# Desilo/liberate-fhe

Measured on AMD Instinct MI355X. Metric: NTTs/sec (forward negacyclic poly-NTT, logN=16, L=30 limbs, bit-exact vs reference semantics), higher is better.
Workload: dtype int64; 1 GPU; gold preset (logN=16), rows 9..38 of the prime chain (25 scale + base + 4 special primes = 30 limbs), 128 polynomials per GPU per step, forward NTT via lf_ntt_ws (C ABI: lf_ntt through a resident workspace of the operands' size); workspace_bytes=2013511680, batch_per_gpu=128, limbs=30, logN=16, parallelism=replicas x1 (independent polynomials)

## Files before the change

liberate_fhe_amd/csrc/ckks_ntt_core.h:

```cpp
#pragma once
#include "ckks_common.h"
#include <stdlib.h>

#define NTT_THREADS 512
#define NTT_PASS_WAVES 6
#define NTT_LDS_WORDS ((1 << NTT_TILE_LOG_MAX) + (1 << (NTT_TILE_LOG_MAX - 3)))
#define TAIL_NONE (-1)
#define SMALL_PRIME_LIMIT (1ull << SMALL_PRIME_BITS)

#define PAD(L) ((L) + ((L) >> 3))
#define PAD_STRIDE(LOGDL) ((1 << (LOGDL)) + ((1 << (LOGDL)) >> 3))
#define NTT_FLAG_WORD NTT_LDS_WORDS

namespace {

__device__ __forceinline__ int lf_tid() {
    const int wave = __builtin_amdgcn_readfirstlane((int)threadIdx.x >> 6);
    int lane;
    asm volatile("v_mbcnt_lo_u32_b32 %0, -1, 0\n\tv_mbcnt_hi_u32_b32 %0, -1, %0" : "=v"(lane));
    return (wave << 6) | lane;
}

__device__ __forceinline__ void lds_barrier() {
    asm volatile("s_waitcnt lgkmcnt(0)" ::: "memory");
// ... 512 lines not shown
    int s = g.s0, left = g.S, log_d = g.strided ? g.logC : 0;
    Ctx cc = c;
    int nstep = 0;
    auto arm = [&](int K) {
        ++nstep;
        cc.inv_reduce = ((nstep & 1) == 0) || (left - K <= 0);
    };
    if (FAST && g.tl == 12 && g.S == 12) {
        StepTwInv<A, 0> t0;
        StepTwInv<A, 3> t3;
        StepTwInv<A, 6> t6;
        StepTwInv<A, 9> t9;
        t0.load(c, s, adj, g.logN, base, lf_tid());
        arm(3); inv_step8<A, 0>(sm, t0, cc, lf_tid()); left -= 3;
        t3.load(c, s + 3, adj, g.logN, base, lf_tid());
        lds_barrier();
        arm(3); inv_step8<A, 3>(sm, t3, cc, lf_tid()); left -= 3;
        t6.load(c, s + 6, adj, g.logN, base, lf_tid());
        lds_barrier();
        arm(3); inv_step8<A, 6>(sm, t6, cc, lf_tid()); left -= 3;
        t9.load(c, s + 9, adj, g.logN, base, lf_tid());
        lds_barrier();
        arm(3); inv_step8<A, 9>(sm, t9, cc, lf_tid());
        lds_barrier();
        return;
    }
    while (left > 0) {
        if (FAST && left >= 3) {
            arm(3);
            inv_step<3, A>(sm, T, log_d, s, adj, g.logN, base, cc);
            s += 3; left -= 3; log_d += 3;
        } else if (FAST && left == 2) {
            arm(2);
            inv_step<2, A>(sm, T, log_d, s, adj, g.logN, base, cc);
            s += 2; left -= 2; log_d += 2;
        } else {
            arm(1);
            inv_step<1, A>(sm, T, log_d, s, adj, g.logN, base, cc);
            s += 1; left -= 1; log_d += 1;
        }
        lds_barrier();
    }
}

__device__ __forceinline__ RowDp make_dp_tab(const RowMod &m, const double *__restrict__ tw_dp) {
    RowDp d;
    d.q = (double)m.q;
    d.q2 = 2.0 * d.q;
    d.qinv = tw_dp[0];
    d.q2inv = 0.5 * d.qinv;
    return d;
}

__device__ __forceinline__ RowDp make_dp(const RowMod &m) {
    RowDp d;
    d.q = (double)m.q;
    d.q2 = 2.0 * d.q;
    d.qinv = 1.0 / d.q;
    d.q2inv = 0.5 * d.qinv;
    return d;
}

__device__ __forceinline__ void store_tile_raw(const i64 *sm, i64 *row, const PassGeom &g, int tile) {
    const int T = 1 << g.tl;
    for (int L = threadIdx.x * 2; L < T; L += NTT_THREADS * 2) {
        longlong2 v;
        v.x = sm[PAD(L)];
        v.y = sm[PAD(L + 1)];
        store_tile_pair(row, g, tile, L, v);
    }
}

static_assert(NTT_THREADS == 512, "one flag byte per wave fills the 8-byte flag word");

__device__ __forceinline__ void wave_flag_set(i64 *sm, int pred) {
    const bool any = __builtin_amdgcn_ballot_w64(pred != 0) != 0;
    const int t = lf_tid();
    if ((t & 63) == 0) reinterpret_cast<unsigned char *>(sm + NTT_FLAG_WORD)[t >> 6] = any ? 1 : 0;
}

__device__ __forceinline__ void wave_lds_sync() {
    asm volatile("s_waitcnt lgkmcnt(0)" ::: "memory");
    __builtin_amdgcn_wave_barrier();
}

#define LF_TID(KEEP, w0) ((KEEP) ? (w0) : lf_tid())
template <class A, bool KEEP, bool CHECK>
__device__ __forceinline__ bool fwd_tile12_core(typename A::T *smt, i64 *sm, typename A::T (&x)[8], int s, int E, int base,
                                                const Ctx &c, int w0) {
    StepTw<A, 9> t9;
    StepTw<A, 6> t6;
    StepTw<A, 3> t3;
    StepTw<A, 0> t0;
    t9.load(c, s, E, base, LF_TID(KEEP, w0));
    fwd_regs8<A, 9>(x, t9, c);
    {
        typename A::T *sp = smt + PAD(LF_TID(KEEP, w0));
#pragma unroll
        for (int e = 0; e < 8; ++e) sp[e * PAD_STRIDE(9)] = x[e];
    }
    t6.load(c, s + 3, E, base, LF_TID(KEEP, w0));
    lds_barrier();
    if (CHECK && sm[NTT_FLAG_WORD] != 0) {
        lds_barrier();
        return false;
    }
// ... 1081 lines not shown
```

liberate_fhe_amd/csrc/ckks_ntt_tile16.h:

```cpp
#pragma once
#include "ckks_ntt_core.h"

#define NTT16_THREADS 256
#define PAD16(L) ((L) + ((L) >> 4))
#define NTT16_LDS_WORDS (4096 + 256)
#define NTT16_FLAG NTT16_LDS_WORDS

namespace {

template <class A>
struct Tw16Early {
    typename A::W w1[1], w2[2], w4[4];
    __device__ __forceinline__ void load(const Ctx &c, int i) {
        A::tw_group(c, i, 1, w1);
        A::tw_group(c, i << 1, 2, w2);
        A::tw_group(c, i << 2, 4, w4);
    }
    __device__ __forceinline__ void get(int cnt, typename A::W (&wv)[8]) const {
#pragma unroll
        for (int j = 0; j < 4; ++j)
            if (j < cnt) wv[j] = cnt == 1 ? w1[0] : (cnt == 2 ? w2[j & 1] : w4[j]);
    }
};

template <class A>
struct Tw16Last {
    typename A::W w8[8];
    __device__ __forceinline__ void load(const Ctx &c, int i) { A::tw_group(c, i << 3, 8, w8); }
};

template <class A, int U0 = 0>
__device__ __forceinline__ void fwd_regs16(typename A::T (&x)[16], int i0, const Ctx &c, const Tw16Early<A> *early = nullptr,
                                           const Tw16Last<A> *last = nullptr) {
#pragma unroll
    for (int u = U0; u < 4; ++u) {
        const int du = 1 << (3 - u);
        typename A::W wv[8];
        if (early && u < 3) early->get(1 << u, wv);
        else if (last && u == 3) {
#pragma unroll
            for (int j = 0; j < 8; ++j) wv[j] = last->w8[j];
        } else A::tw_group(c, i0 << u, 1 << u, wv);
#pragma unroll
        for (int j = 0; j < (1 << u); ++j) {
            const int e0 = j << (4 - u);
#pragma unroll
            for (int t = 0; t < du; ++t) A::fwd(c, x[e0 + t], x[e0 + t + du], wv[j], (i0 << u) + j);
        }
    }
    A::fwd_end(c, x);
}

template <int U0 = 0>
__device__ __forceinline__ void fwd_regs16_exact(double (&x)[16], int i0, const Ctx &c, const Tw16Early<ArithDp> *early = nullptr,
                                                 const Tw16Last<ArithDp> *last = nullptr) {
#pragma unroll
    for (int u = U0; u < 4; ++u) {
        const int du = 1 << (3 - u);
        double wv[8];
        if (early && u < 3) early->get(1 << u, wv);
        else if (last && u == 3) {
#pragma unroll
            for (int j = 0; j < 8; ++j) wv[j] = last->w8[j];
        } else ArithDp::tw_group(c, i0 << u, 1 << u, wv);
        double V[8];
#pragma unroll
        for (int j = 0; j < (1 << u); ++j) {
            const int e0 = j << (4 - u);
#pragma unroll
            for (int t = 0; t < du; ++t) V[j * du + t] = dp_mulmod(x[e0 + t + du], wv[j], c.d);
        }
        int hmin = min(min(__double2hiint(V[0]), __double2hiint(V[1])), __double2hiint(V[2]));
        hmin = min(min(hmin, __double2hiint(V[3])), __double2hiint(V[4]));
        hmin = min(min(hmin, __double2hiint(V[5])), __double2hiint(V[6]));
        hmin = min(hmin, __double2hiint(V[7]));
        if (__builtin_expect(__builtin_amdgcn_ballot_w64(hmin < 0x41500000) != 0, 0)) {
#pragma unroll
            for (int j = 0; j < (1 << u); ++j) {
                const int e0 = j << (4 - u);
#pragma unroll
                for (int t = 0; t < du; ++t) {
                    double &v = V[j * du + t];
                    if (dp_below_fix_limit(v))
                        v = dp_lazy_fix(v, (u64)c.tw_mont[(i0 << u) + j], (u64)dp_reduce(x[e0 + t + du], c.d.q2, c.d.q2inv), c.d.q);
                }
            }
        }
#pragma unroll
        for (int j = 0; j < (1 << u); ++j) {
            const int e0 = j << (4 - u);
#pragma unroll
            for (int t = 0; t < du; ++t) {
                const double U = x[e0 + t], Vv = V[j * du + t];
                x[e0 + t] = U + Vv;
                x[e0 + t + du] = U - Vv;
            }
        }
    }
}

template <class A>
__device__ __forceinline__ void inv_regs16(typename A::T (&x)[16], int il, const Ctx &c, const Tw16Early<A> *early = nullptr) {
#pragma unroll
    for (int u = 0; u < 4; ++u) {
        const int du = 1 << u;
        typename A::W wv[8];
        if (early && u > 0) early->get(1 << (3 - u), wv);
        else A::tw_group(c, il << (3 - u), 1 << (3 - u), wv);
#pragma unroll
        for (int h = 0; h < (1 << (3 - u)); ++h) {
            const int e0 = h << (u + 1);
#pragma unroll
            for (int t = 0; t < du; ++t) A::inv(c, x[e0 + t], x[e0 + t + du], wv[h], (il << (3 - u)) + h);
// ... 43 lines not shown
                const int k = h * du + t;
                x[e0 + t] = x[e0 + t] + x[e0 + t + du];
                x[e0 + t + du] = V[k];
            }
        }
    }
#pragma unroll
    for (int e = 0; e < 16; ++e) x[e] = dp_reduce(x[e], c.d.q2, c.d.q2inv);
}

__device__ __forceinline__ void tile16_slow_compute(i64 *sm, int base, int s0, int logN, bool inverse, const Ctx &c, int j0 = 0,
                                                    int j1 = 12) {
    for (int j = j0; j < j1; ++j) {
        const int st = s0 + j;
        const int logd = inverse ? j : 11 - j;
        for (int i = threadIdx.x; i < 2048; i += NTT16_THREADS) {
            const int pa = ((i >> logd) << (logd + 1)) | (i & ((1 << logd) - 1)), pb = pa + (1 << logd);
            i64 a = sm[PAD16(pa)], b = sm[PAD16(pb)];
            if (!inverse) {
                const int idx = (1 << st) + ((base + pa) >> (logN - st));
                ArithInt<true>::fwd(c, a, b, c.tw_mont[idx], idx);
            } else {
                const int idx = (1 << (logN - st - 1)) + ((base + pa) >> (st + 1));
                ArithInt<true>::inv(c, a, b, c.tw_mont[idx], idx);
            }
            sm[PAD16(pa)] = a;
            sm[PAD16(pb)] = b;
        }
        __syncthreads();
    }
}
__device__ __forceinline__ void tile16_slow_lds(i64 *sm, i64 *dst, int base, int s0, int logN, bool inverse, const Ctx &c, int j0 = 0,
                                                int j1 = 12) {
    tile16_slow_compute(sm, base, s0, logN, inverse, c, j0, j1);
    for (int L = threadIdx.x; L < 4096; L += NTT16_THREADS) dst[L] = sm[PAD16(L)];
}
__device__ __forceinline__ void tile16_slow(i64 *sm, const i64 *src, i64 *dst, int base, int s0, int logN, bool inverse, const Ctx &c) {
    for (int L = threadIdx.x; L < 4096; L += NTT16_THREADS) sm[PAD16(L)] = src[L];
    __syncthreads();
    tile16_slow_lds(sm, dst, base, s0, logN, inverse, c);
}

__device__ __forceinline__ void wave_flag_set16(i64 *sm, int pred, int w) {
    const bool any = __builtin_amdgcn_ballot_w64(pred != 0) != 0;
    if ((w & 63) == 0) reinterpret_cast<unsigned char *>(sm + NTT16_FLAG)[w >> 6] = any ? 1 : 0;
}
__device__ __forceinline__ bool tile_flagged16(const i64 *sm) { return reinterpret_cast<const unsigned *>(sm + NTT16_FLAG)[0] != 0; }

template <bool RLX> struct DpArith { typedef ArithDp type; };
template <> struct DpArith<true> { typedef ArithDpR type; };

template <class A, bool EXACT_DP, int U0 = 0>
__device__ __forceinline__ void fwd_step16(typename A::T (&x)[16], int i0, const Ctx &c, const Tw16Early<A> *early,
                                           const Tw16Last<A> *last = nullptr) {
    if constexpr (EXACT_DP) fwd_regs16_exact<U0>(x, i0, c, early, last);
    else fwd_regs16<A, U0>(x, i0, c, early, last);
}
template <class A, bool EXACT_DP>
__device__ __forceinline__ void inv_step16(typename A::T (&x)[16], int il, const Ctx &c, const Tw16Early<A> *early) {
    if constexpr (EXACT_DP) inv_regs16_exact(x, il, c, early);
    else inv_regs16<A>(x, il, c, early);
}

template <class A, bool DP, bool RLX, int U0 = 0>
__device__ __forceinline__ bool fwd_tile16_steps(typename A::T *smt, const i64 *sm, typename A::T (&x)[16], int w, int base,
                                                 int E, int s, const Ctx &c, bool check, const Tw16Last<A> *lastC = nullptr) {
    constexpr bool EX = DP && !RLX;
    const int iA = (1 << s) + (base >> (E - s));
    const int pB = ((w >> 4) << 8) | (w & 15);
    const int iB = (1 << (s + 4)) + ((base + pB) >> (E - s - 4));
    const int iC = (1 << (s + 8)) + ((base + 16 * w) >> (E - s - 8));
    Tw16Early<A> twB, twC;
    fwd_step16<A, EX, U0>(x, iA, c, nullptr);
    {
        typename A::T *sp = smt + PAD16(w);
#pragma unroll
        for (int e = 0; e < 16; ++e) sp[e * 272] = x[e];
    }
    twB.load(c, iB);
    lds_barrier();
    if (check && tile_flagged16(sm)) return false;
    {
        typename A::T *sp = smt + PAD16(pB);
#pragma unroll
        for (int e = 0; e < 16; ++e) x[e] = sp[e * 17];
        fwd_step16<A, EX>(x, iB, c, &twB);
#pragma unroll
        for (int e = 0; e < 16; ++e) sp[e * 17] = x[e];
    }
    twC.load(c, iC);
    lds_barrier();
    {
        const typename A::T *sp = smt + 17 * w;
#pragma unroll
        for (int e = 0; e < 16; ++e) x[e] = sp[e];
    }
    fwd_step16<A, EX>(x, iC, c, &twC, lastC);
    return true;
}

template <bool DP, bool RLX> struct FwdArith { typedef ArithInt<false> type; };
template <> struct FwdArith<true, false> { typedef ArithDp type; };
template <> struct FwdArith<true, true> { typedef ArithDpR type; };
template <> struct FwdArith<false, true> { typedef ArithShoup type; };

template <bool DP, bool RLX, bool PLN = false>
__device__ __forceinline__ void fwd_tile16(i64 *sm, i64 *__restrict__ row, int tile, const PassGeom &g, const Ctx &c,
                                           const Tw16Last<typename FwdArith<DP, RLX>::type> *lastC = nullptr) {
    static_assert(!PLN || (DP && RLX), "planes: relaxed fp64-class rows only");
    const int w = lf_tid();
    const int base = tile << 12, E = g.logN, s = g.s0;
    constexpr bool CHECK = !RLX;
    constexpr bool NTL = RLX ? NT_RLOAD : NT_EXACT, NTS = RLX ? NT_RSTORE : NT_EXACT;
    i64 raw[16];
    unsigned plo[PLN ? 16 : 1];
    unsigned short phi[PLN ? 16 : 1];
    if constexpr (PLN) {
        const unsigned *lo = reinterpret_cast<const unsigned *>(row) + base;
        const unsigned short *hi = reinterpret_cast<const unsigned short *>(row + ((i64)1 << (E - 1))) + base;
#pragma unroll
        for (int e = 0; e < 16; ++e) {
            plo[e] = __builtin_nontemporal_load(uniform_at(lo + (e << 8), (unsigned)w));
            phi[e] = __builtin_nontemporal_load(uniform_at(hi + (e << 8), (unsigned)w));
        }
    } else {
#pragma unroll
        for (int e = 0; e < 16; ++e) {
            if constexpr (NTL) raw[e] = __builtin_nontemporal_load(uniform_at(row + base + (e << 8), (unsigned)w));
            else raw[e] = *uniform_at(row + base + (e << 8), (unsigned)w);
        }
    }
    if (CHECK) {
        int odd = 0;
#pragma unroll
        for (int e = 0; e < 16; ++e) odd |= ((u64)raw[e] >= (u64)c.m.q2);
        wave_flag_set16(sm, odd, w);
    }
    i64 o[16];
    bool ok;
    if constexpr (DP) {
        typedef typename DpArith<RLX>::type AD;
        double x[16];
#pragma unroll
        for (int e = 0; e < 16; ++e) x[e] = PLN ? dp_from_planes(plo[e], phi[e]) : RLX ? dp_from_signed(raw[e]) : dp_from_word(raw[e]);
        ok = fwd_tile16_steps<AD, true, RLX>(reinterpret_cast<double *>(sm), sm, x, w, base, E, s, c, CHECK, lastC);
        const double md = RLX ? c.d.q : c.d.q2, mi = RLX ? c.d.qinv : c.d.q2inv;
#pragma unroll
        for (int e = 0; e < 16; ++e) o[e] = dp_to_word(dp_reduce(x[e], md, mi));
    } else if constexpr (RLX) {
        ok = fwd_tile16_steps<ArithShoup, false, true>(sm, sm, raw, w, base, E, s, c, false, lastC);
#pragma unroll
        for (int e = 0; e < 16; ++e) o[e] = ArithShoup::canon(c, raw[e]);
    } else {
        ok = fwd_tile16_steps<ArithInt<false>, false, RLX>(sm, sm, raw, w, base, E, s, c, true, lastC);
#pragma unroll
        for (int e = 0; e < 16; ++e) o[e] = raw[e];
    }
    if (!ok) {
        __syncthreads();
        tile16_slow(sm, row + base, row + base, base, s, E, false, c);
        return;
    }
    if constexpr (PLN) {
        const int lane = w & 63, wave = w >> 6;
        unsigned *sw = reinterpret_cast<unsigned *>(sm + 17 * 64 * wave);
#pragma unroll
        for (int k = 0; k < 4; ++k) {
            const lf_u4_t v = {(unsigned)o[4 * k], (unsigned)o[4 * k + 1], (unsigned)o[4 * k + 2], (unsigned)o[4 * k + 3]};
            *reinterpret_cast<lf_u4_t *>(sw + lane * 20 + 4 * k) = v;
        }
#pragma unroll
        for (int k = 0; k < 2; ++k) {
            lf_u4_t v;
#pragma unroll
            for (int m = 0; m < 4; ++m)
                v[m] = (unsigned)(o[8 * k + 2 * m] >> 32) | ((unsigned)(o[8 * k + 2 * m + 1] >> 32) << 16);
            *reinterpret_cast<lf_u4_t *>(sw + 1280 + lane * 12 + 4 * k) = v;
        }
        wave_lds_sync();
        unsigned *lo = reinterpret_cast<unsigned *>(row) + base + (wave << 10);
        unsigned *hi = reinterpret_cast<unsigned *>(row + ((i64)1 << (E - 1))) + ((base + (wave << 10)) >> 1);
#pragma unroll
        for (int i = 0; i < 4; ++i) {
            const lf_u4_t v = *reinterpret_cast<const lf_u4_t *>(sw + (16 * i + (lane >> 2)) * 20 + 4 * (lane & 3));
            *reinterpret_cast<lf_u4_t *>(lo + (i << 8) + 4 * lane) = v;
        }
#pragma unroll
        for (int i = 0; i < 2; ++i) {
            const lf_u4_t v = *reinterpret_cast<const lf_u4_t *>(sw + 1280 + (32 * i + (lane >> 1)) * 12 + 4 * (lane & 1));
            *reinterpret_cast<lf_u4_t *>(hi + (i << 8) + 4 * lane) = v;
        }
        return;
    }
    {
        i64 *sp = sm + 17 * w;
#pragma unroll
        for (int e = 0; e < 16; ++e) sp[e] = o[e];
    }
    wave_lds_sync();
    const int L0 = ((w >> 6) << 10) + ((w & 63) << 1);
    const i64 *so = sm + PAD16(L0);
#pragma unroll
    for (int i = 0; i < 8; ++i) {
        longlong2 v;
        v.x = so[i * 136];
        v.y = so[i * 136 + 1];
        if constexpr (NTS) nt_store2(row + base + L0 + (i << 7), v);
        else *reinterpret_cast<longlong2 *>(row + base + L0 + (i << 7)) = v;
    }
}

template <bool DP, bool SKIP0>
__device__ __forceinline__ bool ws_load_tile(const i64 *__restrict__ srow, const unsigned char *__restrict__ wf, int base, int E,
                                             int w, i64 (&raw)[16]) {
    const int wave = __builtin_amdgcn_readfirstlane(w >> 6);
    w = (int)lane_here((unsigned)w, srow);
    const u64 *fp = reinterpret_cast<const u64 *>(wf + (wave << 4));
    const u64 fl = fp[0], fh = SKIP0 ? fp[0] : fp[1];
    if constexpr (DP) {
        const unsigned *lo = reinterpret_cast<const unsigned *>(srow) + base;
        const unsigned short *mid = reinterpret_cast<const unsigned short *>(srow + ((i64)1 << (E - 1))) + base;
#pragma unroll
        for (int e = 0; e < 16; ++e) {
            const unsigned l = __builtin_nontemporal_load(uniform_at(lo + (e << 8), (unsigned)w));
            const unsigned m = __builtin_nontemporal_load(uniform_at(mid + (e << 8), (unsigned)w));
            raw[e] = (i64)(((u64)m << 32) | (u64)l);
        }
        if ((fl | fh) != 0) {
            const unsigned short *top = reinterpret_cast<const unsigned short *>(srow + 3 * ((i64)1 << (E - 2))) + base;
#pragma unroll
            for (int e = 0; e < 16; ++e)
                if ((((e < 8 ? fl : fh) >> (8 * (e & 7))) & 0xffull) != 0) raw[e] |= (i64)((u64)top[(e << 8) + w] << 48);
        }
    } else {
#pragma unroll
        for (int e = 0; e < 16; ++e) raw[e] = __builtin_nontemporal_load(uniform_at(srow + base + (e << 8), (unsigned)w));
    }
    return (fl | fh) != 0;
}

template <bool DP, bool SKIP0>
__device__ __forceinline__ void fwd_tile16_ws(i64 *sm, const i64 *__restrict__ srow, const unsigned char *__restrict__ wf,
                                              i64 *__restrict__ row, int tile, const PassGeom &g, const Ctx &c,
                                              const Tw16Last<typename FwdArith<DP, false>::type> *lastC = nullptr) {
    const int w = lf_tid();
    const int base = tile << 12, E = g.logN, s = g.s0;
    i64 raw[16];
    const bool flagged = ws_load_tile<DP, SKIP0>(srow, wf, base, E, w, raw);
    {
        int odd = 0;
        if (flagged) {
#pragma unroll
            for (int e = 0; e < 16; ++e) odd |= ((u64)raw[e] >= (u64)c.m.q2);
        }
        wave_flag_set16(sm, odd, w);
    }
    i64 o[16];
    bool ok;
    if constexpr (DP) {
        double x[16];
#pragma unroll
        for (int e = 0; e < 16; ++e) x[e] = dp_from_word(raw[e]);
        ok = fwd_tile16_steps<ArithDp, true, false, SKIP0 ? 1 : 0>(reinterpret_cast<double *>(sm), sm, x, w, base, E, s, c, true, lastC);
#pragma unroll
        for (int e = 0; e < 16; ++e) o[e] = dp_to_word(dp_reduce(x[e], c.d.q2, c.d.q2inv));
    } else {
        ok = fwd_tile16_steps<ArithInt<false>, false, false, SKIP0 ? 1 : 0>(sm, sm, raw, w, base, E, s, c, true, lastC);
#pragma unroll
        for (int e = 0; e < 16; ++e) o[e] = raw[e];
    }
    if (!ok) {
        __syncthreads();
        ws_load_tile<DP, SKIP0>(srow, wf, base, E, w, raw);
#pragma unroll
        for (int e = 0; e < 16; ++e) sm[PAD16(w + (e << 8))] = raw[e];
        __syncthreads();
        tile16_slow_lds(sm, row + base, base, s, E, false, c, SKIP0 ? 1 : 0);
        return;
    }
    {
        i64 *sp = sm + 17 * w;
#pragma unroll
        for (int e = 0; e < 16; ++e) sp[e] = o[e];
    }
    wave_lds_sync();
    const int L0 = ((w >> 6) << 10) + ((w & 63) << 1);
    const i64 *so = sm + PAD16(L0);
#pragma unroll
    for (int i = 0; i < 8; ++i) {
        longlong2 v;
        v.x = so[i * 136];
        v.y = so[i * 136 + 1];
        if constexpr (NT_EXACT) nt_store2(row + base + L0 + (i << 7), v);
        else *reinterpret_cast<longlong2 *>(row + base + L0 + (i << 7)) = v;
    }
}

template <class A, bool DP, bool RLX>
__device__ __forceinline__ bool inv_tile16_steps(typename A::T *smt, const i64 *sm, typename A::T (&x)[16], int w, int base,
                                                 int logN, int s, const Ctx &c, bool check) {
    constexpr bool EX = DP && !RLX;
    const int iC = (1 << (logN - s - 4)) + ((base + 16 * w) >> (s + 4));
    const int pB = ((w >> 4) << 8) | (w & 15);
    const int iB = (1 << (logN - s - 8)) + ((base + pB) >> (s + 8));
    const int iA = (1 << (logN - s - 12)) + (base >> (s + 12));
    Tw16Early<A> twB;
    inv_step16<A, EX>(x, iC, c, nullptr);
    {
        typename A::T *sp = smt + 17 * w;
#pragma unroll
        for (int e = 0; e < 16; ++e) sp[e] = x[e];
    }
    twB.load(c, iB);
    lds_barrier();
    if (check && tile_flagged16(sm)) return false;
    {
        typename A::T *sp = smt + PAD16(pB);
#pragma unroll
        for (int e = 0; e < 16; ++e) x[e] = sp[e * 17];
        inv_step16<A, EX>(x, iB, c, &twB);
// ... 293 lines not shown
                                                                            const i64 *__restrict__ kl, const i64 *__restrict__ kh) {
    __shared__ i64 sm[NTT16_LDS_WORDS + 1];
    const int b = blockIdx.x;
    if (b < cl.in_blocks) {
        if (b < cl.in_real) pass16_body<false, true, false>(sm, b, dst, dst, g, cl.in, tw_br, tw_dp, ql, qh, kl, kh);
    } else {
        pass16_body<true, true, false, false, PLN_IN | PLN_OUT>(sm, b - cl.in_blocks, dst, dst, g, cl.dp, tw_br, tw_dp, ql, qh, kl, kh);
    }
}

__global__ void __launch_bounds__(NTT16_THREADS, 4) ntt_pass16_inv_planes(const i64 *src, i64 *dst, PassGeom g, ClassLists cl,
                                                                            const i64 *__restrict__ tw_br,
                                                                            const double *__restrict__ tw_dp,
                                                                            const i64 *__restrict__ ql, const i64 *__restrict__ qh,
                                                                            const i64 *__restrict__ kl, const i64 *__restrict__ kh) {
    __shared__ i64 sm[NTT16_LDS_WORDS + 1];
    const int b = blockIdx.x;
    if (b < cl.in_blocks) {
        if (b < cl.in_real) pass16_body<false, true, true>(sm, b, src, dst, g, cl.in, tw_br, tw_dp, ql, qh, kl, kh);
    } else {
        pass16_body<true, true, true, false, PLN_IN | PLN_OUT>(sm, b - cl.in_blocks, src, dst, g, cl.dp, tw_br, tw_dp, ql, qh, kl, kh);
    }
}

__global__ void __launch_bounds__(NTT16_THREADS, 4) ntt_pass16_mul_planes(const i64 *src, i64 *dst, PassGeom g, ClassLists cl, MulSrc ms,
                                                                            const i64 *__restrict__ tw_br,
                                                                            const double *__restrict__ tw_dp,
                                                                            const i64 *__restrict__ ql, const i64 *__restrict__ qh,
                                                                            const i64 *__restrict__ kl, const i64 *__restrict__ kh) {
    __shared__ i64 sm[NTT16_LDS_WORDS + 1];
    const int b = blockIdx.x;
    if (b < cl.in_blocks) {
        if (b < cl.in_real) pass16_body<false, true, true, true>(sm, b, src, dst, g, cl.in, tw_br, tw_dp, ql, qh, kl, kh, &ms);
    } else {
        pass16_body<true, true, true, true, PLN_IN>(sm, b - cl.in_blocks, src, dst, g, cl.dp, tw_br, tw_dp, ql, qh, kl, kh, &ms);
    }
}

__global__ void __launch_bounds__(NTT16_THREADS, 4) ntt_pass16_mul_mixed(const i64 *src, i64 *dst, PassGeom g, ClassLists cl, MulSrc ms,
                                                                           const i64 *__restrict__ tw_br,
                                                                           const double *__restrict__ tw_dp,
                                                                           const i64 *__restrict__ ql, const i64 *__restrict__ qh,
                                                                           const i64 *__restrict__ kl, const i64 *__restrict__ kh) {
    __shared__ i64 sm[NTT16_LDS_WORDS + 1];
    const int b = blockIdx.x;
    if (b < cl.in_blocks) {
        if (b < cl.in_real) pass16_body<false, true, true, true>(sm, b, src, dst, g, cl.in, tw_br, tw_dp, ql, qh, kl, kh, &ms);
    } else {
        pass16_body<true, true, true, true>(sm, b - cl.in_blocks, src, dst, g, cl.dp, tw_br, tw_dp, ql, qh, kl, kh, &ms);
    }
}

struct TileAt {
    int live, poly, crow, tile;
};
__device__ __forceinline__ TileAt tile_at(const PassGeom &g, const RowList &rl, int b, bool live) {
    TileAt t;
    t.live = 0, t.poly = 0, t.crow = 0, t.tile = 0;
    if (!live) return t;
    const int tiles = 1 << (g.logN - g.tl);
    const int pairs = rl.n * tiles;
    int pair, poly;
    if ((pairs & 7) == 0) {
        const int r = b >> 3;
        poly = r % g.batch;
        pair = (r / g.batch) * 8 + (b & 7);
    } else {
        pair = b / g.batch;
        poly = b % g.batch;
    }
    pair = __builtin_amdgcn_readfirstlane(pair);
    t.poly = __builtin_amdgcn_readfirstlane(poly);
    const int li = pair >> (g.logN - g.tl);
    t.crow = (int)((reinterpret_cast<const unsigned *>(rl.id)[li >> 1] >> ((li & 1) << 4)) & 0xffffu);
    t.tile = pair & (tiles - 1);
    t.live = 1;
    return t;
}

template <bool DP, bool RLX>
__device__ __forceinline__ void seq16_loop(i64 *sm, i64 *dst, const PassGeom &g, const RowList &rl, int b0, int bend, int tpb,
                                           const i64 *__restrict__ tw_br, const double *__restrict__ tw_dp,
                                           const i64 *__restrict__ ql, const i64 *__restrict__ qh,
                                           const i64 *__restrict__ kl, const i64 *__restrict__ kh) {
    typedef typename FwdArith<DP, RLX>::type AC;
    const int w = lf_tid();
    Tw16Last<AC> last;
    int last_crow = -1, last_tile = -1;
    for (int i = 0; i < tpb; ++i) {
        const int b = b0 + 8 * i;
        const TileAt t = tile_at(g, rl, b, b < bend);
        if (!t.live) break;
        Ctx c;
        c.m = load_mod(ql, qh, kl, kh, t.crow);
        c.tw_mont = tw_br + ((i64)t.crow << g.logN);
        set_aux<DP>(c, tw_dp, t.crow, g.logN);
        c.d = DP ? make_dp_tab(c.m, c.tw_dp) : make_dp(c.m);
        c.relaxed = RLX ? 1 : 0;
        c.inv_reduce = 0;
        if (t.crow != last_crow || t.tile != last_tile) {
            last.load(c, (1 << (g.s0 + 8)) + (((t.tile << 12) + 16 * w) >> (g.logN - g.s0 - 8)));
            last_crow = t.crow, last_tile = t.tile;
        }
        if (i) lds_barrier();
        fwd_tile16<DP, RLX>(sm, dst + ((i64)(t.poly * g.rows + t.crow) << g.logN), t.tile, g, c, &last);
    }
}

template <bool RLX>
__global__ void __launch_bounds__(NTT16_THREADS, 4) ntt_pass16_fwd_seq(i64 *dst, PassGeom g, ClassLists cl, int total, int tpb,
                                                                         const i64 *__restrict__ tw_br,
                                                                         const double *__restrict__ tw_dp,
                                                                         const i64 *__restrict__ ql, const i64 *__restrict__ qh,
                                                                         const i64 *__restrict__ kl, const i64 *__restrict__ kh) {
    __shared__ i64 sm[NTT16_LDS_WORDS + 1];
    const int vb0 = (int)(blockIdx.x & 7) + 8 * (int)(blockIdx.x >> 3) * tpb;
    if (vb0 < cl.in_blocks) seq16_loop<false, RLX>(sm, dst, g, cl.in, vb0, cl.in_real, tpb, tw_br, tw_dp, ql, qh, kl, kh);
    else seq16_loop<true, RLX>(sm, dst, g, cl.dp, vb0 - cl.in_blocks, total - cl.in_blocks, tpb, tw_br, tw_dp, ql, qh, kl, kh);
}

template <bool DP> struct TilePf;
template <> struct TilePf<true> {
    unsigned lo[16];
    unsigned short mid[16];
};
template <> struct TilePf<false> {
    i64 raw[16];
};

template <bool DP, bool SKIP0>
__device__ __forceinline__ bool ws_prefetch_tile(const i64 *__restrict__ srow, const unsigned char *__restrict__ wf, int base, int E, int w,
                                                 TilePf<DP> &pf) {
    const int wave = __builtin_amdgcn_readfirstlane(w >> 6);
    w = (int)lane_here((unsigned)w, srow);
    const u64 *fp = reinterpret_cast<const u64 *>(wf + (wave << 4));
    const u64 fl = fp[0], fh = SKIP0 ? fp[0] : fp[1];
    if constexpr (DP) {
        const unsigned *lo = reinterpret_cast<const unsigned *>(srow) + base;
        const unsigned short *mid = reinterpret_cast<const unsigned short *>(srow + ((i64)1 << (E - 1))) + base;
#pragma unroll
        for (int e = 0; e < 16; ++e) {
            pf.lo[e] = __builtin_nontemporal_load(uniform_at(lo + (e << 8), (unsigned)w));
            pf.mid[e] = __builtin_nontemporal_load(uniform_at(mid + (e << 8), (unsigned)w));
        }
    } else {
#pragma unroll
        for (int e = 0; e < 16; ++e) pf.raw[e] = __builtin_nontemporal_load(uniform_at(srow + base + (e << 8), (unsigned)w));
    }
    return (fl | fh) != 0;
}

template <bool DP, bool SKIP0>
__device__ __forceinline__ void fwd_tile16_ws_pf(i64 *sm, TilePf<DP> &pf, bool &pf_flagged, const i64 *__restrict__ srow,
                                                  const unsigned char *__restrict__ wf, i64 *__restrict__ row, int tile,
                                                  const PassGeom &g, const Ctx &c, const Tw16Last<typename FwdArith<DP, false>::type> *lastC,
                                                  const i64 *__restrict__ nsrow, const unsigned char *__restrict__ nwf, int ntile) {
    const int w = lf_tid();
    const int base = tile << 12, E = g.logN, s = g.s0;
    i64 raw[16];
    const bool flagged = pf_flagged;
    if (flagged) {
        ws_load_tile<DP, SKIP0>(srow, wf, base, E, w, raw);
    } else if constexpr (DP) {
#pragma unroll
        for (int e = 0; e < 16; ++e) raw[e] = (i64)(((u64)pf.mid[e] << 32) | (u64)pf.lo[e]);
    } else {
#pragma unroll
        for (int e = 0; e < 16; ++e) raw[e] = pf.raw[e];
    }
    {
        int odd = 0;
        if (flagged) {
#pragma unroll
            for (int e = 0; e < 16; ++e) odd |= ((u64)raw[e] >= (u64)c.m.q2);
        }
        wave_flag_set16(sm, odd, w);
    }
    i64 o[16];
    bool ok;
    if constexpr (DP) {
        double x[16];
#pragma unroll
        for (int e = 0; e < 16; ++e) x[e] = dp_from_word(raw[e]);
        ok = fwd_tile16_steps<ArithDp, true, false, SKIP0 ? 1 : 0>(reinterpret_cast<double *>(sm), sm, x, w, base, E, s, c, true, lastC);
#pragma unroll
        for (int e = 0; e < 16; ++e) o[e] = dp_to_word(dp_reduce(x[e], c.d.q2, c.d.q2inv));
    } else {
        ok = fwd_tile16_steps<ArithInt<false>, false, false, SKIP0 ? 1 : 0>(sm, sm, raw, w, base, E, s, c, true, lastC);
#pragma unroll
        for (int e = 0; e < 16; ++e) o[e] = raw[e];
    }
    if (!ok) {
        __syncthreads();
        ws_load_tile<DP, SKIP0>(srow, wf, base, E, w, raw);
#pragma unroll
        for (int e = 0; e < 16; ++e) sm[PAD16(w + (e << 8))] = raw[e];
        __syncthreads();
        tile16_slow_lds(sm, row + base, base, s, E, false, c, SKIP0 ? 1 : 0);
        if (ntile >= 0) pf_flagged = ws_prefetch_tile<DP, SKIP0>(nsrow, nwf, ntile << 12, E, w, pf);
        else pf = TilePf<DP>{};
        return;
    }

    {
        i64 *sp = sm + 17 * w;
#pragma unroll
        for (int e = 0; e < 16; ++e) sp[e] = o[e];
    }
    __builtin_amdgcn_sched_barrier(0);
    if (ntile >= 0) pf_flagged = ws_prefetch_tile<DP, SKIP0>(nsrow, nwf, ntile << 12, E, w, pf);
    else pf = TilePf<DP>{};
    __builtin_amdgcn_sched_barrier(0);
    wave_lds_sync();
    const int L0 = ((w >> 6) << 10) + ((w & 63) << 1);
    const i64 *so = sm + PAD16(L0);
#pragma unroll
    for (int i = 0; i < 8; ++i) {
        longlong2 v;
        v.x = so[i * 136];
        v.y = so[i * 136 + 1];
        if constexpr (NT_EXACT) nt_store2(row + base + L0 + (i << 7), v);
        else *reinterpret_cast<longlong2 *>(row + base + L0 + (i << 7)) = v;
    }
}

#ifndef NTT16_WS_PREFETCH
#define NTT16_WS_PREFETCH 1
#endif

template <bool DP, bool SKIP0>
__device__ __forceinline__ void seq16_loop_ws(i64 *sm, const i64 *ws, const unsigned char *wflags, i64 *dst, const PassGeom &g,
                                              const RowList &rl, int b0, int bend, int tpb, const i64 *__restrict__ tw_br,
                                              const double *__restrict__ tw_dp, const i64 *__restrict__ ql,
                                              const i64 *__restrict__ qh, const i64 *__restrict__ kl, const i64 *__restrict__ kh) {
    typedef typename FwdArith<DP, false>::type AC;
    const int w = lf_tid();
    Tw16Last<AC> last;
    int last_crow = -1, last_tile = -1;
#if NTT16_WS_PREFETCH
    TilePf<DP> pf;
    bool pf_flagged = false;
    TileAt t = tile_at(g, rl, b0, b0 < bend);
    if (!t.live) return;
    {
        const i64 ri = (i64)(t.poly * g.rows + t.crow);
        pf_flagged = ws_prefetch_tile<DP, SKIP0>(ws + (ri << g.logN), wflags + (ri << 6), t.tile << 12, g.logN, w, pf);
    }
    for (int i = 0; i < tpb; ++i) {
        const int bn = b0 + 8 * (i + 1);
        TileAt tn = tile_at(g, rl, bn, i + 1 < tpb && bn < bend);
        Ctx c;
        c.m = load_mod(ql, qh, kl, kh, t.crow);
        c.tw_mont = tw_br + ((i64)t.crow << g.logN);
        set_aux<DP>(c, tw_dp, t.crow, g.logN);
        c.d = DP ? make_dp_tab(c.m, c.tw_dp) : make_dp(c.m);
        c.relaxed = 0;
        c.inv_reduce = 0;
        if (t.crow != last_crow || t.tile != last_tile) {
            last.load(c, (1 << (g.s0 + 8)) + (((t.tile << 12) + 16 * w) >> (g.logN - g.s0 - 8)));
            last_crow = t.crow, last_tile = t.tile;
        }
        if (i) lds_barrier();
        const i64 ri = (i64)(t.poly * g.rows + t.crow), rn = (i64)(tn.poly * g.rows + tn.crow);
        fwd_tile16_ws_pf<DP, SKIP0>(sm, pf, pf_flagged, ws + (ri << g.logN), wflags + (ri << 6), dst + (ri << g.logN), t.tile, g, c, &last,
                                    ws + (rn << g.logN), wflags + (rn << 6), tn.live ? tn.tile : -1);
        if (!tn.live) break;
        t = tn;
    }
#else
    for (int i = 0; i < tpb; ++i) {
        const int b = b0 + 8 * i;
        const TileAt t = tile_at(g, rl, b, b < bend);
        if (!t.live) break;
        Ctx c;
        c.m = load_mod(ql, qh, kl, kh, t.crow);
        c.tw_mont = tw_br + ((i64)t.crow << g.logN);
        set_aux<DP>(c, tw_dp, t.crow, g.logN);
        c.d = DP ? make_dp_tab(c.m, c.tw_dp) : make_dp(c.m);
        c.relaxed = 0;
        c.inv_reduce = 0;
        if (t.crow != last_crow || t.tile != last_tile) {
            last.load(c, (1 << (g.s0 + 8)) + (((t.tile << 12) + 16 * w) >> (g.logN - g.s0 - 8)));
            last_crow = t.crow, last_tile = t.tile;
        }
        if (i) lds_barrier();
        const i64 ri = (i64)(t.poly * g.rows + t.crow);
        fwd_tile16_ws<DP, SKIP0>(sm, ws + (ri << g.logN), wflags + (ri << 6), dst + (ri << g.logN), t.tile, g, c, &last);
    }
#endif
}

template <bool SKIP0>
__global__ void __launch_bounds__(NTT16_THREADS, 4) ntt_pass16_fwd_seq_ws(const i64 *ws, const unsigned char *wflags, i64 *dst,
                                                                            PassGeom g, ClassLists cl, int total, int tpb,
                                                                            const i64 *__restrict__ tw_br,
                                                                            const double *__restrict__ tw_dp,
                                                                            const i64 *__restrict__ ql, const i64 *__restrict__ qh,
                                                                            const i64 *__restrict__ kl, const i64 *__restrict__ kh) {
    __shared__ i64 sm[NTT16_LDS_WORDS + 1];
    const int vb0 = (int)(blockIdx.x & 7) + 8 * (int)(blockIdx.x >> 3) * tpb;
    if (vb0 < cl.in_blocks) seq16_loop_ws<false, SKIP0>(sm, ws, wflags, dst, g, cl.in, vb0, cl.in_real, tpb, tw_br, tw_dp, ql, qh, kl, kh);
    else seq16_loop_ws<true, SKIP0>(sm, ws, wflags, dst, g, cl.dp, vb0 - cl.in_blocks, total - cl.in_blocks, tpb, tw_br, tw_dp, ql, qh, kl, kh);
}

template <bool DP, bool SKIP0>
__device__ __forceinline__ void pass16_ws_body(i64 *sm, int b, const i64 *ws, const unsigned char *wflags, i64 *dst,
                                               const PassGeom &g, const RowList &rl, const i64 *__restrict__ tw_br,
                                               const double *__restrict__ tw_dp, const i64 *__restrict__ ql,
                                               const i64 *__restrict__ qh, const i64 *__restrict__ kl, const i64 *__restrict__ kh) {
    int poly, crow, tile;
    block_coords(g, rl, b, poly, crow, tile);
    poly = __builtin_amdgcn_readfirstlane(poly), crow = __builtin_amdgcn_readfirstlane(crow);
    tile = __builtin_amdgcn_readfirstlane(tile);
    Ctx c;
    c.m = load_mod(ql, qh, kl, kh, crow);
    c.tw_mont = tw_br + ((i64)crow << g.logN);
    set_aux<DP>(c, tw_dp, crow, g.logN);
    c.d = DP ? make_dp_tab(c.m, c.tw_dp) : make_dp(c.m);
    c.relaxed = 0;
    c.inv_reduce = 0;
    const i64 ri = (i64)(poly * g.rows + crow);
    fwd_tile16_ws<DP, SKIP0>(sm, ws + (ri << g.logN), wflags + (ri << 6), dst + (ri << g.logN), tile, g, c);
}

template <bool SKIP0>
__global__ void __launch_bounds__(NTT16_THREADS, 4) ntt_pass16_fwd_ws(const i64 *ws, const unsigned char *wflags, i64 *dst,
                                                                        PassGeom g, ClassLists cl, const i64 *__restrict__ tw_br,
                                                                        const double *__restrict__ tw_dp,
                                                                        const i64 *__restrict__ ql, const i64 *__restrict__ qh,
                                                                        const i64 *__restrict__ kl, const i64 *__restrict__ kh) {
    __shared__ i64 sm[NTT16_LDS_WORDS + 1];
    const int b = blockIdx.x;
    if (b < cl.in_blocks) {
        if (b < cl.in_real) pass16_ws_body<false, SKIP0>(sm, b, ws, wflags, dst, g, cl.in, tw_br, tw_dp, ql, qh, kl, kh);
    } else {
        pass16_ws_body<true, SKIP0>(sm, b - cl.in_blocks, ws, wflags, dst, g, cl.dp, tw_br, tw_dp, ql, qh, kl, kh);
    }
}

template <bool DP, bool RLX, bool INV>
__global__ void __launch_bounds__(NTT16_THREADS, 4) ntt_pass16(const i64 *src, i64 *dst, PassGeom g, RowList rl,
                                                                const i64 *__restrict__ tw_br, const double *__restrict__ tw_dp,
// ... 98 lines not shown
```

Measured before the change: 82100 poly-NTT/s.

## Cache per-row context and step-A twiddles across tiles with incremental tile walk

Replaces the per-iteration divide/modulo tile lookup with an incremental walker that advances poly and pair by constants, and recomputes row coordinates only when the pair changes. The per-row Ctx (modulus, dp constants, twiddle pointers) is now loaded only on a new pair for exact rows. First-stage twiddles are fetched once per pair into one 32-bit half per lane and broadcast with readlane. The dp constants are built by exponent bit manipulation instead of a convert and divide. These cut scalar integer divisions, redundant global loads and twiddle fetches in the sequential tile loops, at the cost of readlane traffic and extra live registers.

```diff
diff --git a/liberate_fhe_amd/csrc/ckks_ntt_core.h b/liberate_fhe_amd/csrc/ckks_ntt_core.h
--- a/liberate_fhe_amd/csrc/ckks_ntt_core.h
+++ b/liberate_fhe_amd/csrc/ckks_ntt_core.h
@@ -588,6 +588,18 @@
     return d;
 }
 
+__device__ __forceinline__ RowDp make_dp_tab_uniform(const RowMod &m, const double *__restrict__ tw_dp) {
+    const int k = 63 - __builtin_clzll(m.q);
+    const u64 qb = ((u64)(1023 + k) << 52) | ((m.q << (52 - k)) & 0x000FFFFFFFFFFFFFull);
+    const u64 ib = (u64)__double_as_longlong(tw_dp[0]);
+    RowDp d;
+    d.q = __longlong_as_double((i64)qb);
+    d.q2 = __longlong_as_double((i64)(qb + (1ull << 52)));
+    d.qinv = __longlong_as_double((i64)ib);
+    d.q2inv = __longlong_as_double((i64)(ib - (1ull << 52)));
+    return d;
+}
+
 __device__ __forceinline__ RowDp make_dp(const RowMod &m) {
     RowDp d;
     d.q = (double)m.q;
diff --git a/liberate_fhe_amd/csrc/ckks_ntt_tile16.h b/liberate_fhe_amd/csrc/ckks_ntt_tile16.h
--- a/liberate_fhe_amd/csrc/ckks_ntt_tile16.h
+++ b/liberate_fhe_amd/csrc/ckks_ntt_tile16.h
@@ -1,5 +1,7 @@
 #pragma once
 #include "ckks_ntt_core.h"
+#include "ckks_tile_walk.h"
+#include <type_traits>
 
 #define NTT16_THREADS 256
 #define PAD16(L) ((L) + ((L) >> 4))
@@ -29,14 +31,37 @@
     __device__ __forceinline__ void load(const Ctx &c, int i) { A::tw_group(c, i << 3, 8, w8); }
 };
 
+template <class A>
+struct Tw16StepA {
+    unsigned half;
+    __device__ __forceinline__ void load(const Ctx &c, int i, int w) {
+        static_assert(sizeof(typename A::W) == 8, "8-byte table entries");
+        const unsigned m = min((unsigned)(w & 31) + 1u, 15u);
+        const int u = 31 - __builtin_clz(m);
+        const typename A::W v = A::tw(c, (i << u) + (int)(m ^ (1u << u)));
+        const u64 bits = *reinterpret_cast<const u64 *>(&v);
+        half = (w & 32) ? (unsigned)(bits >> 32) : (unsigned)bits;
+    }
+    __device__ __forceinline__ void get(int u, typename A::W (&wv)[8]) const {
+#pragma unroll
+        for (int j = 0; j < 8; ++j)
+            if (sizeof(typename A::W) == 8 && j < (1 << u)) {
+                const int lane = (1 << u) - 1 + j;
+                const u64 bits = ((u64)(unsigned)__builtin_amdgcn_readlane((int)half, 32 + lane) << 32) | (unsigned)__builtin_amdgcn_readlane((int)half, lane);
+                __builtin_memcpy(&wv[j], &bits, 8);
+            }
+    }
+};
+
 template <class A, int U0 = 0>
 __device__ __forceinline__ void fwd_regs16(typename A::T (&x)[16], int i0, const Ctx &c, const Tw16Early<A> *early = nullptr,
-                                           const Tw16Last<A> *last = nullptr) {
+                                           const Tw16Last<A> *last = nullptr, const Tw16StepA<A> *stA = nullptr) {
 #pragma unroll
     for (int u = U0; u < 4; ++u) {
         const int du = 1 << (3 - u);
         typename A::W wv[8];
-        if (early && u < 3) early->get(1 << u, wv);
+        if (stA) stA->get(u, wv);
+        else if (early && u < 3) early->get(1 << u, wv);
         else if (last && u == 3) {
 #pragma unroll
             for (int j = 0; j < 8; ++j) wv[j] = last->w8[j];
@@ -53,12 +78,13 @@
 
 template <int U0 = 0>
 __device__ __forceinline__ void fwd_regs16_exact(double (&x)[16], int i0, const Ctx &c, const Tw16Early<ArithDp> *early = nullptr,
-                                                 const Tw16Last<ArithDp> *last = nullptr) {
+                                                 const Tw16Last<ArithDp> *last = nullptr, const Tw16StepA<ArithDp> *stA = nullptr) {
 #pragma unroll
     for (int u = U0; u < 4; ++u) {
         const int du = 1 << (3 - u);
         double wv[8];
-        if (early && u < 3) early->get(1 << u, wv);
+        if (stA) stA->get(u, wv);
+        else if (early && u < 3) early->get(1 << u, wv);
         else if (last && u == 3) {
 #pragma unroll
             for (int j = 0; j < 8; ++j) wv[j] = last->w8[j];
@@ -208,9 +234,9 @@
 
 template <class A, bool EXACT_DP, int U0 = 0>
 __device__ __forceinline__ void fwd_step16(typename A::T (&x)[16], int i0, const Ctx &c, const Tw16Early<A> *early,
-                                           const Tw16Last<A> *last = nullptr) {
-    if constexpr (EXACT_DP) fwd_regs16_exact<U0>(x, i0, c, early, last);
-    else fwd_regs16<A, U0>(x, i0, c, early, last);
+                                           const Tw16Last<A> *last = nullptr, const Tw16StepA<A> *stA = nullptr) {
+    if constexpr (EXACT_DP) fwd_regs16_exact<U0>(x, i0, c, early, last, stA);
+    else fwd_regs16<A, U0>(x, i0, c, early, last, stA);
 }
 template <class A, bool EXACT_DP>
 __device__ __forceinline__ void inv_step16(typename A::T (&x)[16], int il, const Ctx &c, const Tw16Early<A> *early) {
@@ -220,14 +246,15 @@
 
 template <class A, bool DP, bool RLX, int U0 = 0>
 __device__ __forceinline__ bool fwd_tile16_steps(typename A::T *smt, const i64 *sm, typename A::T (&x)[16], int w, int base,
-                                                 int E, int s, const Ctx &c, bool check, const Tw16Last<A> *lastC = nullptr) {
+                                                 int E, int s, const Ctx &c, bool check, const Tw16Last<A> *lastC = nullptr,
+                                                 const Tw16StepA<A> *stA = nullptr) {
     constexpr bool EX = DP && !RLX;
     const int iA = (1 << s) + (base >> (E - s));
     const int pB = ((w >> 4) << 8) | (w & 15);
     const int iB = (1 << (s + 4)) + ((base + pB) >> (E - s - 4));
     const int iC = (1 << (s + 8)) + ((base + 16 * w) >> (E - s - 8));
     Tw16Early<A> twB, twC;
-    fwd_step16<A, EX, U0>(x, iA, c, nullptr);
+    fwd_step16<A, EX, U0>(x, iA, c, nullptr, nullptr, stA);
     {
         typename A::T *sp = smt + PAD16(w);
 #pragma unroll
@@ -262,7 +289,8 @@
 
 template <bool DP, bool RLX, bool PLN = false>
 __device__ __forceinline__ void fwd_tile16(i64 *sm, i64 *__restrict__ row, int tile, const PassGeom &g, const Ctx &c,
-                                           const Tw16Last<typename FwdArith<DP, RLX>::type> *lastC = nullptr) {
+                                           const Tw16Last<typename FwdArith<DP, RLX>::type> *lastC = nullptr,
+                                           const Tw16StepA<typename FwdArith<DP, RLX>::type> *stA = nullptr) {
     static_assert(!PLN || (DP && RLX), "planes: relaxed fp64-class rows only");
     const int w = lf_tid();
     const int base = tile << 12, E = g.logN, s = g.s0;
@@ -299,7 +327,7 @@
         double x[16];
 #pragma unroll
         for (int e = 0; e < 16; ++e) x[e] = PLN ? dp_from_planes(plo[e], phi[e]) : RLX ? dp_from_signed(raw[e]) : dp_from_word(raw[e]);
-        ok = fwd_tile16_steps<AD, true, RLX>(reinterpret_cast<double *>(sm), sm, x, w, base, E, s, c, CHECK, lastC);
+        ok = fwd_tile16_steps<AD, true, RLX>(reinterpret_cast<double *>(sm), sm, x, w, base, E, s, c, CHECK, lastC, stA);
         const double md = RLX ? c.d.q : c.d.q2, mi = RLX ? c.d.qinv : c.d.q2inv;
 #pragma unroll
         for (int e = 0; e < 16; ++e) o[e] = dp_to_word(dp_reduce(x[e], md, mi));
@@ -308,7 +336,7 @@
 #pragma unroll
         for (int e = 0; e < 16; ++e) o[e] = ArithShoup::canon(c, raw[e]);
     } else {
-        ok = fwd_tile16_steps<ArithInt<false>, false, RLX>(sm, sm, raw, w, base, E, s, c, true, lastC);
+        ok = fwd_tile16_steps<ArithInt<false>, false, RLX>(sm, sm, raw, w, base, E, s, c, true, lastC, stA);
 #pragma unroll
         for (int e = 0; e < 16; ++e) o[e] = raw[e];
     }
@@ -398,7 +426,8 @@
 template <bool DP, bool SKIP0>
 __device__ __forceinline__ void fwd_tile16_ws(i64 *sm, const i64 *__restrict__ srow, const unsigned char *__restrict__ wf,
                                               i64 *__restrict__ row, int tile, const PassGeom &g, const Ctx &c,
-                                              const Tw16Last<typename FwdArith<DP, false>::type> *lastC = nullptr) {
+                                              const Tw16Last<typename FwdArith<DP, false>::type> *lastC = nullptr,
+                                              const Tw16StepA<typename FwdArith<DP, false>::type> *stA = nullptr) {
     const int w = lf_tid();
     const int base = tile << 12, E = g.logN, s = g.s0;
     i64 raw[16];
@@ -417,11 +446,11 @@
         double x[16];
 #pragma unroll
         for (int e = 0; e < 16; ++e) x[e] = dp_from_word(raw[e]);
-        ok = fwd_tile16_steps<ArithDp, true, false, SKIP0 ? 1 : 0>(reinterpret_cast<double *>(sm), sm, x, w, base, E, s, c, true, lastC);
+        ok = fwd_tile16_steps<ArithDp, true, false, SKIP0 ? 1 : 0>(reinterpret_cast<double *>(sm), sm, x, w, base, E, s, c, true, lastC, stA);
 #pragma unroll
         for (int e = 0; e < 16; ++e) o[e] = dp_to_word(dp_reduce(x[e], c.d.q2, c.d.q2inv));
     } else {
-        ok = fwd_tile16_steps<ArithInt<false>, false, false, SKIP0 ? 1 : 0>(sm, sm, raw, w, base, E, s, c, true, lastC);
+        ok = fwd_tile16_steps<ArithInt<false>, false, false, SKIP0 ? 1 : 0>(sm, sm, raw, w, base, E, s, c, true, lastC, stA);
 #pragma unroll
         for (int e = 0; e < 16; ++e) o[e] = raw[e];
     }
@@ -821,58 +850,89 @@
 }
 
 struct TileAt {
-    int live, poly, crow, tile;
+    int live, poly, crow, tile, pair;
 };
-__device__ __forceinline__ TileAt tile_at(const PassGeom &g, const RowList &rl, int b, bool live) {
-    TileAt t;
-    t.live = 0, t.poly = 0, t.crow = 0, t.tile = 0;
-    if (!live) return t;
-    const int tiles = 1 << (g.logN - g.tl);
-    const int pairs = rl.n * tiles;
-    int pair, poly;
-    if ((pairs & 7) == 0) {
-        const int r = b >> 3;
-        poly = r % g.batch;
-        pair = (r / g.batch) * 8 + (b & 7);
-    } else {
-        pair = b / g.batch;
-        poly = b % g.batch;
-    }
-    pair = __builtin_amdgcn_readfirstlane(pair);
-    t.poly = __builtin_amdgcn_readfirstlane(poly);
+__device__ __forceinline__ void pair_coords(const PassGeom &g, const RowList &rl, int pair, TileAt &t) {
     const int li = pair >> (g.logN - g.tl);
     t.crow = (int)((reinterpret_cast<const unsigned *>(rl.id)[li >> 1] >> ((li & 1) << 4)) & 0xffffu);
-    t.tile = pair & (tiles - 1);
+    t.tile = pair & ((1 << (g.logN - g.tl)) - 1);
+    t.pair = pair;
+}
+__device__ __forceinline__ TileAt tile_at(const PassGeom &g, const RowList &rl, int b, bool live, TileWalk &wk) {
+    TileAt t;
+    t.live = 0, t.poly = 0, t.crow = 0, t.tile = 0, t.pair = -1;
+    wk = TileWalk{};
+    if (!live) return t;
+    const int pairs = rl.n << (g.logN - g.tl);
+    wk = tile_walk_start(b, g.batch, (pairs & 7) == 0);
+    wk.poly = __builtin_amdgcn_readfirstlane(wk.poly), wk.pair = __builtin_amdgcn_readfirstlane(wk.pair);
+    wk.dq = __builtin_amdgcn_readfirstlane(wk.dq), wk.dr = __builtin_amdgcn_readfirstlane(wk.dr);
+    t.poly = wk.poly;
+    pair_coords(g, rl, wk.pair, t);
     t.live = 1;
     return t;
 }
+__device__ __forceinline__ TileAt tile_next(const PassGeom &g, const RowList &rl, const TileAt &t, bool live, TileWalk &wk) {
+    TileAt n;
+    n.live = 0, n.poly = 0, n.crow = 0, n.tile = 0, n.pair = -1;
+    if (!live) return n;
+    wk = tile_walk_next(wk, g.batch);
+    n = t;
+    n.poly = wk.poly;
+    if (wk.pair != t.pair) pair_coords(g, rl, wk.pair, n);
+    return n;
+}
+
+template <bool DP, bool RLX>
+struct Seq16Kept {
+    typedef typename FwdArith<DP, RLX>::type AC;
+    struct None {};
+    Ctx c;
+    typename std::conditional<RLX, None, Tw16StepA<AC>>::type stA;
+    Tw16Last<AC> last;
+    int pair = -1;
+    __device__ __forceinline__ void load_ctx(const PassGeom &g, const TileAt &t, const i64 *__restrict__ tw_br,
+                                             const double *__restrict__ tw_dp, const i64 *__restrict__ ql, const i64 *__restrict__ qh,
+                                             const i64 *__restrict__ kl, const i64 *__restrict__ kh) {
+        c.m = load_mod(ql, qh, kl, kh, t.crow);
+        c.tw_mont = tw_br + ((i64)t.crow << g.logN);
+        set_aux<DP>(c, tw_dp, t.crow, g.logN);
+        c.d = DP ? (RLX ? make_dp_tab(c.m, c.tw_dp) : make_dp_tab_uniform(c.m, c.tw_dp)) : make_dp(c.m);
+        c.relaxed = RLX ? 1 : 0;
+        c.inv_reduce = 0;
+    }
+    __device__ __forceinline__ void enter(const PassGeom &g, const TileAt &t, int w, const i64 *__restrict__ tw_br,
+                                          const double *__restrict__ tw_dp, const i64 *__restrict__ ql, const i64 *__restrict__ qh,
+                                          const i64 *__restrict__ kl, const i64 *__restrict__ kh) {
+        const bool fresh = t.pair != pair;
+        if (RLX || fresh) load_ctx(g, t, tw_br, tw_dp, ql, qh, kl, kh);
+        if (fresh) {
+            const int base = t.tile << 12;
+            if constexpr (!RLX) stA.load(c, (1 << g.s0) + (base >> (g.logN - g.s0)), w);
+            last.load(c, (1 << (g.s0 + 8)) + ((base + 16 * w) >> (g.logN - g.s0 - 8)));
+            pair = t.pair;
+        }
+    }
+    __device__ __forceinline__ const Tw16StepA<AC> *step_a() const {
+        if constexpr (RLX) return nullptr;
+        else return &stA;
+    }
+};
 
 template <bool DP, bool RLX>
 __device__ __forceinline__ void seq16_loop(i64 *sm, i64 *dst, const PassGeom &g, const RowList &rl, int b0, int bend, int tpb,
                                            const i64 *__restrict__ tw_br, const double *__restrict__ tw_dp,
                                            const i64 *__restrict__ ql, const i64 *__restrict__ qh,
                                            const i64 *__restrict__ kl, const i64 *__restrict__ kh) {
-    typedef typename FwdArith<DP, RLX>::type AC;
     const int w = lf_tid();
-    Tw16Last<AC> last;
-    int last_crow = -1, last_tile = -1;
-    for (int i = 0; i < tpb; ++i) {
-        const int b = b0 + 8 * i;
-        const TileAt t = tile_at(g, rl, b, b < bend);
-        if (!t.live) break;
-        Ctx c;
-        c.m = load_mod(ql, qh, kl, kh, t.crow);
-        c.tw_mont = tw_br + ((i64)t.crow << g.logN);
-        set_aux<DP>(c, tw_dp, t.crow, g.logN);
-        c.d = DP ? make_dp_tab(c.m, c.tw_dp) : make_dp(c.m);
-        c.relaxed = RLX ? 1 : 0;
-        c.inv_reduce = 0;
-        if (t.crow != last_crow || t.tile != last_tile) {
-            last.load(c, (1 << (g.s0 + 8)) + (((t.tile << 12) + 16 * w) >> (g.logN - g.s0 - 8)));
-            last_crow = t.crow, last_tile = t.tile;
-        }
+    Seq16Kept<DP, RLX> k;
+    TileWalk wk;
+    TileAt t = tile_at(g, rl, b0, b0 < bend, wk);
+    for (int i = 0; i < tpb && t.live; ++i) {
+        k.enter(g, t, w, tw_br, tw_dp, ql, qh, kl, kh);
         if (i) lds_barrier();
-        fwd_tile16<DP, RLX>(sm, dst + ((i64)(t.poly * g.rows + t.crow) << g.logN), t.tile, g, c, &last);
+        fwd_tile16<DP, RLX>(sm, dst + ((i64)(t.poly * g.rows + t.crow) << g.logN), t.tile, g, k.c, &k.last, k.step_a());
+        t = tile_next(g, rl, t, i + 1 < tpb && b0 + 8 * (i + 1) < bend, wk);
     }
 }
 
@@ -923,6 +983,7 @@
 __device__ __forceinline__ void fwd_tile16_ws_pf(i64 *sm, TilePf<DP> &pf, bool &pf_flagged, const i64 *__restrict__ srow,
                                                   const unsigned char *__restrict__ wf, i64 *__restrict__ row, int tile,
                                                   const PassGeom &g, const Ctx &c, const Tw16Last<typename FwdArith<DP, false>::type> *lastC,
+                                                  const Tw16StepA<typename FwdArith<DP, false>::type> *stA,
                                                   const i64 *__restrict__ nsrow, const unsigned char *__restrict__ nwf, int ntile) {
     const int w = lf_tid();
     const int base = tile << 12, E = g.logN, s = g.s0;
@@ -951,11 +1012,11 @@
         double x[16];
 #pragma unroll
         for (int e = 0; e < 16; ++e) x[e] = dp_from_word(raw[e]);
-        ok = fwd_tile16_steps<ArithDp, true, false, SKIP0 ? 1 : 0>(reinterpret_cast<double *>(sm), sm, x, w, base, E, s, c, true, lastC);
+        ok = fwd_tile16_steps<ArithDp, true, false, SKIP0 ? 1 : 0>(reinterpret_cast<double *>(sm), sm, x, w, base, E, s, c, true, lastC, stA);
 #pragma unroll
         for (int e = 0; e < 16; ++e) o[e] = dp_to_word(dp_reduce(x[e], c.d.q2, c.d.q2inv));
     } else {
-        ok = fwd_tile16_steps<ArithInt<false>, false, false, SKIP0 ? 1 : 0>(sm, sm, raw, w, base, E, s, c, true, lastC);
+        ok = fwd_tile16_steps<ArithInt<false>, false, false, SKIP0 ? 1 : 0>(sm, sm, raw, w, base, E, s, c, true, lastC, stA);
 #pragma unroll
         for (int e = 0; e < 16; ++e) o[e] = raw[e];
     }
@@ -1002,61 +1063,34 @@
                                               const RowList &rl, int b0, int bend, int tpb, const i64 *__restrict__ tw_br,
                                               const double *__restrict__ tw_dp, const i64 *__restrict__ ql,
                                               const i64 *__restrict__ qh, const i64 *__restrict__ kl, const i64 *__restrict__ kh) {
-    typedef typename FwdArith<DP, false>::type AC;
     const int w = lf_tid();
-    Tw16Last<AC> last;
-    int last_crow = -1, last_tile = -1;
+    Seq16Kept<DP, false> k;
+    TileWalk wk;
+    TileAt t = tile_at(g, rl, b0, b0 < bend, wk);
+    if (!t.live) return;
 #if NTT16_WS_PREFETCH
     TilePf<DP> pf;
     bool pf_flagged = false;
-    TileAt t = tile_at(g, rl, b0, b0 < bend);
-    if (!t.live) return;
     {
         const i64 ri = (i64)(t.poly * g.rows + t.crow);
         pf_flagged = ws_prefetch_tile<DP, SKIP0>(ws + (ri << g.logN), wflags + (ri << 6), t.tile << 12, g.logN, w, pf);
     }
+#endif
     for (int i = 0; i < tpb; ++i) {
-        const int bn = b0 + 8 * (i + 1);
-        TileAt tn = tile_at(g, rl, bn, i + 1 < tpb && bn < bend);
-        Ctx c;
-        c.m = load_mod(ql, qh, kl, kh, t.crow);
-        c.tw_mont = tw_br + ((i64)t.crow << g.logN);
-        set_aux<DP>(c, tw_dp, t.crow, g.logN);
-        c.d = DP ? make_dp_tab(c.m, c.tw_dp) : make_dp(c.m);
-        c.relaxed = 0;
-        c.inv_reduce = 0;
-        if (t.crow != last_crow || t.tile != last_tile) {
-            last.load(c, (1 << (g.s0 + 8)) + (((t.tile << 12) + 16 * w) >> (g.logN - g.s0 - 8)));
-            last_crow = t.crow, last_tile = t.tile;
-        }
+        const TileAt tn = tile_next(g, rl, t, i + 1 < tpb && b0 + 8 * (i + 1) < bend, wk);
+        k.enter(g, t, w, tw_br, tw_dp, ql, qh, kl, kh);
         if (i) lds_barrier();
-        const i64 ri = (i64)(t.poly * g.rows + t.crow), rn = (i64)(tn.poly * g.rows + tn.crow);
-        fwd_tile16_ws_pf<DP, SKIP0>(sm, pf, pf_flagged, ws + (ri << g.logN), wflags + (ri << 6), dst + (ri << g.logN), t.tile, g, c, &last,
-                                    ws + (rn << g.logN), wflags + (rn << 6), tn.live ? tn.tile : -1);
+        const i64 ri = (i64)(t.poly * g.rows + t.crow);
+#if NTT16_WS_PREFETCH
+        const i64 rn = (i64)(tn.poly * g.rows + tn.crow);
+        fwd_tile16_ws_pf<DP, SKIP0>(sm, pf, pf_flagged, ws + (ri << g.logN), wflags + (ri << 6), dst + (ri << g.logN), t.tile, g, k.c, &k.last,
+                                    k.step_a(), ws + (rn << g.logN), wflags + (rn << 6), tn.live ? tn.tile : -1);
+#else
+        fwd_tile16_ws<DP, SKIP0>(sm, ws + (ri << g.logN), wflags + (ri << 6), dst + (ri << g.logN), t.tile, g, k.c, &k.last, k.step_a());
+#endif
         if (!tn.live) break;
         t = tn;
     }
-#else
-    for (int i = 0; i < tpb; ++i) {
-        const int b = b0 + 8 * i;
-        const TileAt t = tile_at(g, rl, b, b < bend);
-        if (!t.live) break;
-        Ctx c;
-        c.m = load_mod(ql, qh, kl, kh, t.crow);
-        c.tw_mont = tw_br + ((i64)t.crow << g.logN);
-        set_aux<DP>(c, tw_dp, t.crow, g.logN);
-        c.d = DP ? make_dp_tab(c.m, c.tw_dp) : make_dp(c.m);
-        c.relaxed = 0;
-        c.inv_reduce = 0;
-        if (t.crow != last_crow || t.tile != last_tile) {
-            last.load(c, (1 << (g.s0 + 8)) + (((t.tile << 12) + 16 * w) >> (g.logN - g.s0 - 8)));
-            last_crow = t.crow, last_tile = t.tile;
-        }
-        if (i) lds_barrier();
-        const i64 ri = (i64)(t.poly * g.rows + t.crow);
-        fwd_tile16_ws<DP, SKIP0>(sm, ws + (ri << g.logN), wflags + (ri << 6), dst + (ri << g.logN), t.tile, g, c, &last);
-    }
-#endif
 }
 
 template <bool SKIP0>
diff --git a/liberate_fhe_amd/csrc/ckks_tile_walk.h b/liberate_fhe_amd/csrc/ckks_tile_walk.h
--- /dev/null
+++ b/liberate_fhe_amd/csrc/ckks_tile_walk.h
@@ -0,0 +1,37 @@
+#pragma once
+
+#if defined(__HIPCC__)
+#define LF_WALK_FN __host__ __device__ __forceinline__
+#else
+#define LF_WALK_FN static inline
+#endif
+
+typedef struct TileWalk {
+    int poly, pair;
+    int dq, dr, carry;
+} TileWalk;
+
+LF_WALK_FN TileWalk tile_walk_start(int b0, int batch, int xcd) {
+    TileWalk t;
+    if (xcd) {
+        const int r = b0 >> 3;
+        t.poly = r % batch;
+        t.pair = (r / batch) * 8 + (b0 & 7);
+        t.dq = 0, t.dr = 1, t.carry = 8;
+    } else {
+        t.pair = b0 / batch;
+        t.poly = b0 % batch;
+        t.dq = 8 / batch, t.dr = 8 % batch, t.carry = 1;
+    }
+    return t;
+}
+
+LF_WALK_FN TileWalk tile_walk_next(TileWalk t, int batch) {
+    t.poly += t.dr;
+    t.pair += t.dq;
+    if (t.poly >= batch) {
+        t.poly -= batch;
+        t.pair += t.carry;
+    }
+    return t;
+}
```

After: 82000 poly-NTT/s. Within noise of the previous version (-0.1%).
